# Opendigitalradio/ODR-DabMod

Hardware: AMD Instinct MI355X
Metric: Mode-I TX frames/sec (196608 IQ/frame) (higher is better)
Workload: dtype f32; 1 GPU; Mode I full chain from coded bits + GainControl(var) + FIRFilter(45 default taps), native 2.048 Msps (BASELINE config 3); mode=1, prewarm_steps=3, parallelism=1 independent streams

## Files before the change

odr-dabmod_amd/csrc/dabgpu_internal.h:

```cpp
#pragma once

#include <hip/hip_runtime.h>
#include <stddef.h>
#include <stdint.h>

namespace dabgpu {

constexpr int kMaxTaps = 128;
constexpr int kEqTaps = 160;
constexpr int kEqCentre = 56;
constexpr int kMaxTapsUnfused = 512;

struct Geometry {
    int mode;
    int nb_symbols;
    int K;
    int N;
    int logN;
    int null_size;
    int sym_size;
};

struct Tables {
    const float2 *twiddle;
    const uint16_t *src_carrier;
    const uint16_t *dst_pos;
    const uint8_t *phase_q;
    const float *mag;
    const float *taps;
    const float *window;
    const float2 *fir_h;
    const float *eq_g;
};

bool trace_on();
void trace_launch(const char *what);
#define DABGPU_LAUNCH(kernel, ...)                                      \
    do {                                                                \
        if (::dabgpu::trace_on()) ::dabgpu::trace_launch(#kernel);      \
        hipLaunchKernelGGL(kernel, __VA_ARGS__);                        \
    } while (0)

bool streams_overlap(hipStream_t a, hipStream_t b);
hipError_t create_stream_apart(const hipStream_t *others, int n, hipStream_t *out, bool *own);

struct GainParams {
    int mode;
    float constant;
    float var_variance;
    float var_c1;
    float var_c1_lo;
    float var_sq;
};

struct TfArgs {
    Geometry g;
    Tables t;
    GainParams gain;
    int ntaps;
    int n_frames;
    int chunks_per_frame;
    int syms_per_chunk;
    const uint8_t *bits;
    const float2 *carriers;
    float2 *out;
    size_t out_stride;
    float *gain1;
    const float2 *tii_seg;
    int tii_insert0;
    float cfr_clip, cfr_errclip;
    int cfr_mer_base;
    unsigned *cfr_counts;
    double *cfr_mer;
    double *cfr_papr;
    unsigned long long *clipped;
    int overlap;
    unsigned long long *phase_cycles;
};

enum TfFlags { TF_FROM_BITS = 1, TF_GAIN = 2, TF_GUARD = 4, TF_FIR = 8, TF_CFR = 16, TF_GVAR = 32 ,
               TF_OUT_S16 = 64, TF_WINDOW = 256, TF_EQ = 512, TF_OUT_U8 = 1024, TF_OUT_S8 = 2048 };
inline int tf_ofmt(unsigned flags) { return (flags & TF_OUT_S16) ? 1 : (flags & TF_OUT_U8) ? 2 : (flags & TF_OUT_S8) ? 3 : 0; }
inline unsigned tf_ofmt_flag(int fmt) { return fmt == 1 ? TF_OUT_S16 : fmt == 2 ? TF_OUT_U8 : fmt == 3 ? TF_OUT_S8 : 0u; }

hipError_t launch_tf(const TfArgs &a, unsigned flags, hipStream_t s);
size_t tf_lds_bytes(int logN, unsigned flags, int nt = 0, int overlap = 0, int ntaps = 0);
int tf_max_fused_taps();
bool tf_has_eq(const TfArgs &a, unsigned flags);
bool tf_small45(const TfArgs &a, unsigned flags);
bool tf_has_window(const TfArgs &a, unsigned flags);
bool tf_has_fmt(const TfArgs &a, unsigned flags);
bool tf_has_tii(const TfArgs &a, unsigned flags);

hipError_t launch_qpsk(const uint8_t *in, size_t nbytes, int K, float2 *out, hipStream_t s);
hipError_t launch_freq_interleave(const float2 *in, size_t nsamples, int K,
                                  const uint16_t *src_carrier, float2 *out, hipStream_t s);
hipError_t launch_phase_reference(const uint8_t *phase_q, int K, float2 *out, hipStream_t s);
hipError_t launch_diff_mod(const float2 *phase, const float2 *data, size_t nsym_data, int K,
                           float2 *out, hipStream_t s);
hipError_t launch_gain(const float2 *in, size_t nsym, int N, GainParams gp, float2 *out,
                       hipStream_t s);
hipError_t launch_gain_replay(float2 *x0, size_t n_frames, int nsym, int N, GainParams gp, float *gains, float *gain1,
                              bool apply, hipStream_t s);
hipError_t launch_guard_copy(const float2 *in, size_t n_frames, Geometry g, float2 *out,
                             hipStream_t s, const float *gains = nullptr);
hipError_t launch_guard_window(const float2 *in, size_t n_frames, Geometry g, int overlap,
                               const float *window, float2 *out, hipStream_t s, const float *gains = nullptr);
hipError_t launch_guard_fir(const float2 *in, size_t n_frames, Geometry g, int overlap, const float *window,
                            const float *taps, int ntaps, float2 *out, hipStream_t s, const float *gains = nullptr);
hipError_t launch_fir(const float2 *in, size_t frame_samples, size_t n_frames, const float *taps,
                      int ntaps, float2 *out, hipStream_t s);
hipError_t launch_poly(const float2 *in, size_t nsamples, const float *am, const float *pm,
                       float2 *out, hipStream_t s);
hipError_t launch_cic(const float2 *in, size_t nsamples, int K, const float *filter, float2 *out, hipStream_t s);
hipError_t launch_tii(const float2 *in, const uint8_t *acp, int K, int old_variant, int insert, float2 *out,
                      hipStream_t s);
hipError_t launch_tii_add(float2 *out, size_t stride, const float2 *seg, int seg_len, const float *gain1,
                          int insert0, size_t n_frames, hipStream_t s);
hipError_t launch_format(const float *in, size_t nfloats, int fmt, void *out, unsigned long long *clipped,
                         hipStream_t s);
hipError_t launch_lut(const float2 *in, size_t nsamples, float scale, const float *lut,
                      float2 *out, hipStream_t s);

constexpr int kFeCifBytes = 864 * 8;
constexpr int kFeHistory = 15;
struct FeUnit {
    uint32_t in_off, in_bytes;
    uint32_t out_bytes;
    uint32_t dst_off;
    int32_t owner;
    uint32_t nseg;
    uint32_t g0[6], base[6], pat[6];
};
struct FeArgs {
    const uint8_t *eti;
    const uint8_t *prbs;
    const FeUnit *units;
    const int16_t *owner;
    uint8_t *hist;
    uint8_t *fic;
    uint8_t *out;
    int n_eti, n_units, cifs, fic_out;
};
hipError_t launch_fe_encode(const FeArgs &a, hipStream_t s);
hipError_t launch_fe_assemble(const FeArgs &a, hipStream_t s);

struct ResamplerArgs {
    int nin, nout;
    float factor;
    const float *window;
    const float2 *tw_in;
    const float2 *tw_out;
    const float2 *in;
    const float2 *halo;
    float2 *halo_out;
    float2 *out;
    const float *poly;
    unsigned long long *clipped;
    size_t nhops;
    int L, M;
    const float2 *tw_s;
    const float2 *tw_l;
};
hipError_t launch_resampler(const ResamplerArgs &a, hipStream_t s);
bool resampler_has_s16(const ResamplerArgs &a);
// ... 4 lines not shown
```

odr-dabmod_amd/csrc/tf_kernel.h:

```cpp
#pragma once
#include <cstdio>
#include "device_common.h"
#include "tf_layout.h"

namespace dabgpu {
namespace {

constexpr unsigned kCX = 0x901Au;


template <int LOGN> struct ModeGeom;
template <> struct ModeGeom<11> { static constexpr int nb_symbols = 76, K = 1536, null_size = 2656, sym_size = 2552; };
template <> struct ModeGeom<9> { static constexpr int nb_symbols = 76, K = 384, null_size = 664, sym_size = 638; };
template <> struct ModeGeom<8> { static constexpr int nb_symbols = 153, K = 192, null_size = 345, sym_size = 319; };
template <> struct ModeGeom<10> { static constexpr int nb_symbols = 76, K = 768, null_size = 1328, sym_size = 1276; };

template <int LOGN, bool FROM_BITS, bool GAIN, bool GUARD, bool FIR, int NT, bool CFR = false, bool GVAR = false,
          bool ZONLY = false, int OFMT = 0, bool WIN = false, bool EQ = false>
__global__ __launch_bounds__((1 << LOGN) / 8 < 64 ? 64 : (1 << LOGN) / 8,
                             tf_variant(LOGN, FROM_BITS, GAIN, GUARD, FIR, NT, CFR, GVAR, OFMT, WIN, EQ).waves_per_simd)
void tf_kernel(const TfArgs a)
{
    static_assert(!GVAR || (GAIN && !FROM_BITS && !CFR), "GVAR is a specialisation of the carriers path with gain");
    static_assert(!CFR || GUARD == FIR || (FROM_BITS && GUARD),
                  "CFR variants: the full fused epilogue or none of it; the coded-bits chain also with the guard interval alone");
    static_assert(!ZONLY || (LOGN == 11 && GUARD && FIR && NT > 0 && !CFR),
                  "ZONLY: the dual transform of the Mode I chain with the fused FIR");
    static_assert(!ZONLY || FROM_BITS || GVAR || !GAIN, "ZONLY: no gain statistics over the time domain");
    static_assert(!WIN || (FROM_BITS && GUARD && (OFMT == 0 || EQ || (OFMT == 1 && !FIR && !CFR))),
                  "WIN: coded-bits chain with guard interval (integer store: every format with EQ, s16 without FIRFilter)");
    static_assert(!(WIN && FIR) || (!ZONLY && (NT == 0 || (NT == 45 && !CFR)) && !GVAR),
                  "WIN with FIR: the generic packed dual transform (all unfiltered samples at hand), run-time tap count -- or EQ");
    static_assert(!EQ || (FROM_BITS && GUARD && FIR && NT == 45 && !CFR && !GVAR && !ZONLY),
                  "EQ: the coded-bits chain with the 45-tap filter");
    static_assert(!EQ || LOGN == 11 || (LOGN == 10 && !WIN && OFMT == 0),
                  "EQ in transmission mode IV (round 6): complexf output, no windowing (Mode I: WIN with overlap <= kEqWinMax, every format)");
    typedef ModeGeom<LOGN> G;
    typedef Fft<LOGN> F;
    constexpr int N = F::N, T = F::T;
    constexpr TfVariant VAR = tf_variant(LOGN, FROM_BITS, GAIN, GUARD, FIR, NT, CFR, GVAR, OFMT, WIN, EQ);
    constexpr bool CFR_LEAN = VAR.cfr_lean, NOFIR_1BUF = VAR.nofir_1buf, DBUF = VAR.dbuf;
    (void)NOFIR_1BUF;
    constexpr bool HALVES = VAR.halves;
    constexpr int NH = HALVES ? 2 : 1;
    const int t_wg = threadIdx.x;
    const int half = HALVES ? (t_wg >> 5) : 0;
    const int t = HALVES ? (t_wg & 31) : t_wg;
    const bool lane_on = (HALVES || T >= 64) ? true : t < T;
    const unsigned long long on_mask = (HALVES || T >= 64) ? ~0ull : ((1ull << (T & 63)) - 1ull);
    const int tt = lane_on ? t : 0;
    auto hoff = [&](int n) __attribute__((always_inline)) -> int { return HALVES ? half * n : 0; };

    extern __shared__ __attribute__((aligned(16))) char smem[];
    cf *fbuf = reinterpret_cast<cf *>(smem);
    int fpar = 0;
    constexpr bool CFR_SEQ = VAR.cfr_seq;
    constexpr int kXElems = VAR.dual ? 2 * F::LDS_ELEMS : (DBUF ? 2 : 1) * F::LDS_ELEMS;
    double *red = reinterpret_cast<double *>(fbuf + NH * kXElems);
    fbuf += hoff(kXElems);
    uint32_t *phw = reinterpret_cast<uint32_t *>(red + NH * 16);
    red += hoff(16);
    cf *bnd = reinterpret_cast<cf *>(phw + NH * (GAIN ? (FROM_BITS ? T : 6 * T) : 0));
    phw += hoff(T);
    constexpr int KB = NT ? NT - 1 : kBnd;
    cf *wbuf = bnd;
    float *win_l = reinterpret_cast<float *>(wbuf + 6 * kWinMax);
    constexpr int kEqWm = (EQ && WIN) ? kEqWinMax : 0;
    constexpr int kEqQL = kEqTaps - 1 - kEqCentre + kEqWm, kEqQH = 43 + kEqCentre + kEqWm, kEqW = kEqWLen;
    static_assert(kEqQL + kEqQH + 1 + kEqWm <= kEqW && kEqTaps == 160, "EQ window (+ what the unused outputs of a narrower overlap read)");
    static_assert(kEqElems == 3 * kEqW + kEqDLen + (kEqTaps + 8) / 2 + 16 && 2 * kEqWinMax <= 32 && 2 * kEqWinMax + 44 <= 64,
                  "LDS share of the EQ variants (tf_lds_bytes)");
    cf *eq_zp = bnd, *eq_w = bnd + 2 * kEqW, *eq_d = eq_w + kEqW;
    float *g_l = reinterpret_cast<float *>(eq_d + kEqDLen);
    constexpr bool BWIN = VAR.bwin;
    constexpr int kBndElems = 4 * KB + (BWIN ? 4 : 0);
    uint32_t *bitbuf = reinterpret_cast<uint32_t *>(bnd + NH * (EQ ? kEqElems : (FIR && !WIN) ? kBndElems : ((WIN && !FIR) ? 7 * kWinMax : 0)));
    bnd += hoff(kBndElems);
    constexpr int kBitWords = (3 * N / 4) / 16;
    constexpr int kBitStride = kBitWords + 2;
    constexpr bool PAIR = VAR.pair;
    constexpr int kBitBlocks = PAIR ? 4 : 2;
    float *taps_l = reinterpret_cast<float *>(bitbuf + NH * (FROM_BITS ? kBitBlocks * kBitStride : 0));
    bitbuf += hoff(kBitBlocks * kBitStride);
    constexpr int kTapsL = VAR.bwin ? 0 : kMaxTaps, kMagL = 160;
    float *mag_l = taps_l + kTapsL;
    cf *unit8 = reinterpret_cast<cf *>(mag_l + kMagL);
    cf *tw8_l = unit8 + 64;
    F::fill_tw8(a.t.twiddle, tw8_l, t_wg);
    float *cfr_red = reinterpret_cast<float *>(tw8_l + 56);
    uint2 *bsh_l = reinterpret_cast<uint2 *>(cfr_red + 6 * ((T + 63) / 64));
    if (t_wg < 64) {
        const unsigned p = ((unsigned)t_wg + ((unsigned)t_wg >> 3)) & 7u;
        const float cx = (float)((int)((kCX >> (2u * p)) & 3u) - 1);
        const float cy = (float)((int)((kCX >> (2u * ((p + 6u) & 7u))) & 3u) - 1);
        unit8[t_wg] = mk(cx, cy);
    }
    for (int i = t_wg; i < kTapsL; i += blockDim.x) taps_l[i] = FIR ? a.t.taps[i] : 0.f;
    if (EQ)
        for (int i = t; i < kEqTaps + 8; i += blockDim.x) g_l[i] = i < kEqTaps ? a.t.eq_g[i] : 0.f;
    if (EQ) {
        for (int i = t; i < 3 * kEqW + kEqDLen; i += blockDim.x) eq_zp[i] = mk(0.f, 0.f);
    }
    const int W = WIN ? a.overlap : 0;
    constexpr bool kSkipTests = WIN && (FIR || OFMT != 0);
    constexpr int kWm = WIN ? (EQ ? kEqWinMax : (kWinMax < G::sym_size - N ? kWinMax : G::sym_size - N)) : 0;
    const int wfC = (WIN && FIR && !EQ) ? a.ntaps - 1 : 0, wfLP = wfC + 2 * W;
    cf *wfb = tw8_l + 56 + (CFR ? 3 * ((T + 63) / 64) : 0);
    cf *wf_cur = wfb + 2 * wfLP, *wf_U = wf_cur + (2 * W + wfC);
    if (WIN && FIR) win_l = EQ ? g_l + (kEqTaps + 8) : reinterpret_cast<float *>(wf_U + (2 * W + 2 * wfC));
    if (WIN)
        for (int i = t; i < 2 * W; i += blockDim.x) win_l[i] = a.t.window[i];
    if (FROM_BITS)
        for (int i = t_wg; i < G::nb_symbols; i += blockDim.x) mag_l[i] = a.t.mag[i];
    if (BWIN && t < 4) bnd[4 * KB + t] = mk(0.f, 0.f);
    lds_barrier();
    float4 tapa = make_float4(0.f, 0.f, 0.f, 0.f), tapb = tapa, tapc = tapa;
    if constexpr (BWIN) {
        const float4 *tp = reinterpret_cast<const float4 *>(a.t.taps + 12 * (t & 3));
        tapa = tp[0]; tapb = tp[1]; tapc = tp[2];
    }
    const float4 tapm = make_float4((t & 3) == 0 ? 1.f : 0.f, (t & 3) == 1 ? 1.f : 0.f, (t & 3) == 2 ? 1.f : 0.f, (t & 3) == 3 ? 1.f : 0.f);

    constexpr int K = G::K, nsym = G::nb_symbols + 1;
    const int frame0 = NH * (int)(blockIdx.x / a.chunks_per_frame);
    const int chunk = blockIdx.x - (frame0 / NH) * a.chunks_per_frame;
    const bool frame_ok = !HALVES || frame0 + half < a.n_frames;
    const int frame = HALVES ? min(frame0 + half, a.n_frames - 1) : frame0;
    const int s_begin = chunk * a.syms_per_chunk;
    const int s_end = chunk == a.chunks_per_frame - 1 ? nsym : min(nsym, s_begin + a.syms_per_chunk);
    constexpr bool TII_IN = FROM_BITS && GUARD && (EQ || !WIN) && !HALVES;
    const bool tii_on = TII_IN && a.tii_seg != nullptr && s_begin == 0 && (((frame & 1) == 0) == (a.tii_insert0 != 0));
    float g1s = 1.0f;
    if (frame0 >= a.n_frames || s_begin >= nsym) return;

    const int ntaps = NT ? NT : a.ntaps;
    const int C = FIR ? ntaps - 1 : 0;
    constexpr int cp0 = GUARD ? G::null_size - N : 0, cp = GUARD ? G::sym_size - N : 0;
    constexpr int len0 = N + cp0, len = N + cp;

    cf tw[F::NTW > 0 ? F::NTW : 1];
    F::template load_twiddles<true>(a.t.twiddle, tt, tw);

    const int r0 = (tt == 0) ? 3 : 0;
    int kpos[6];
    cf hk[6];
    cf hk8[CFR && FIR ? 8 : 1];
    {
        const int rr[6] = {r0, 1, 2, 5, 6, 7};
#pragma unroll
        for (int c = 0; c < 6; ++c) {
            const int bin = tt + T * rr[c];
            kpos[c] = (bin <= K / 2) ? bin - 1 : bin - N + K;
            if (FIR) hk[c] = a.t.fir_h[bin];
        }
    }
    if (CFR && FIR && !CFR_SEQ) {
#pragma unroll
        for (int m = 0; m < 8; ++m) hk8[m] = a.t.fir_h[tt + T * m];
    }
    int bitpos[6];
    unsigned bsh[6] = {0u, 0u, 0u, 0u, 0u, 0u};
    unsigned P = 0u;
    unsigned fpos[6] = {0u, 4u, 8u, tt == 0 ? 12u : 20u, tt == 0 ? 20u : 16u, tt == 0 ? 16u : 12u};
    const uint8_t *fbits = nullptr;
    if (FROM_BITS) {
        fbits = a.bits + (size_t)frame * (size_t)(G::nb_symbols - 1) * (size_t)(K / 4);
#pragma unroll
        for (int c = 0; c < 6; ++c) {
            bitpos[c] = a.t.src_carrier[kpos[c]];
            bsh[c] = (unsigned)bitpos[c] ^ 7u;
            P |= ((unsigned)a.t.phase_q[kpos[c]] & 3u) << fpos[c];
        }
        if constexpr (CFR_LEAN) {
#pragma unroll
            for (int j = 0; j < 3; ++j) bsh_l[j * T + t] = make_uint2(bsh[2 * j], bsh[2 * j + 1]);
        }
    }
    const cf *fcar = FROM_BITS ? nullptr
                               : a.carriers + (size_t)frame * (size_t)nsym * (size_t)K;
    constexpr int kOutBytes = OFMT == 0 ? 8 : (OFMT == 1 ? 4 : 2);
    const __amdgpu_buffer_rsrc_t orsrc = __builtin_amdgcn_make_buffer_rsrc(
        reinterpret_cast<char *>(a.out) + (size_t)frame0 * a.out_stride * kOutBytes, 0, (int)(NH * a.out_stride * kOutBytes), 0x00020000);
    const int hvoff = HALVES ? (frame_ok ? half * (int)a.out_stride : 0x07ffffff) : 0;
    unsigned nclip = 0;
    typedef unsigned v2u_ __attribute__((ext_vector_type(2)));
#ifdef DABGPU_STORE_AUX
    constexpr int kStoreAux = DABGPU_STORE_AUX;
#else
    constexpr int kStoreAux = (FROM_BITS && LOGN != 8) ? 2 : 0;
#endif
    auto put = [&](int soff, int voff, cf y) __attribute__((always_inline)) {
        if constexpr (OFMT == 1) {
            __builtin_amdgcn_raw_buffer_store_b32(s16_pack(y, nclip), orsrc, voff * 4, soff * 4, kStoreAux);
        } else if constexpr (OFMT == 2 || OFMT == 3) {
            __builtin_amdgcn_raw_buffer_store_b16(b8_pack<(OFMT == 3 ? 3 : 2)>(y, nclip), orsrc, voff * 2, soff * 2, kStoreAux);
        } else {
            const v2u_ d = {__builtin_bit_cast(unsigned, y.x), __builtin_bit_cast(unsigned, y.y)};
            __builtin_amdgcn_raw_buffer_store_b64(d, orsrc, (voff + hvoff) * 8, soff * 8, kStoreAux);
        }
    };

    auto advance = [&](const uint32_t *blk) __attribute__((always_inline)) {
        uint2 w[6];
        unsigned bs[6];
        if constexpr (CFR_LEAN) {
            int tl = t;
            asm volatile("" : "+v"(tl));
#pragma unroll
            for (int j = 0; j < 3; ++j) {
                const uint2 b2 = bsh_l[j * T + tl];
                bs[2 * j] = b2.x;
                bs[2 * j + 1] = b2.y;
            }
        } else {
#pragma unroll
            for (int c = 0; c < 6; ++c) bs[c] = bsh[c];
        }
#pragma unroll
        for (int c = 0; c < 6; ++c)
            w[c] = *reinterpret_cast<const uint2 *>(reinterpret_cast<const char *>(blk) + (__builtin_amdgcn_ubfe(bs[c], 5u, 6u) << 3));
        unsigned I = 0u, Q = 0u;
#pragma unroll
        for (int c = 0; c < 6; ++c) {
            I |= __builtin_amdgcn_ubfe(w[c].x, bs[c], 1u) << fpos[c];
            Q |= __builtin_amdgcn_ubfe(w[c].y, bs[c], 1u) << fpos[c];
        }
        P = (P + ((I ^ Q) | (Q << 1))) & 0x333333u;
    };
    auto fetch_block = [&](int d) __attribute__((always_inline)) -> uint32_t {
        const int dd = min(max(d, 0), G::nb_symbols - 2);
        int tf = t < kBitWords ? t : 0;
        if constexpr (CFR_LEAN) asm volatile("" : "+v"(tf));
        return reinterpret_cast<const uint32_t *>(fbits + (size_t)dd * (size_t)(K / 4))[tf];
    };
    const int bit_slot = t < kBitWords / 2 ? 2 * t : (t < kBitWords ? 2 * (t - kBitWords / 2) + 1 : kBitWords);

    static_assert(!PAIR || (T >= 2 * kBitWords && FROM_BITS), "PAIR: a lane per dword of two blocks");
    auto pair_lane = [&](int &b, int &j, int &slot) __attribute__((always_inline)) {
        int tl = t;
        asm volatile("" : "+v"(tl));
        b = (tl >= kBitWords && tl < 2 * kBitWords) ? 1 : 0;
        j = tl - b * kBitWords;
        slot = tl < 2 * kBitWords ? b * kBitStride + (j < kBitWords / 2 ? 2 * j : 2 * (j - kBitWords / 2) + 1) : kBitWords;
        if (tl >= 2 * kBitWords) j = 0;
    };
    auto fetch_pair = [&](int pr) __attribute__((always_inline)) -> uint32_t {
        int b, j, slot;
        pair_lane(b, j, slot);
        const int blk = min(max(2 * pr + b, 0), G::nb_symbols - 2);
        const uint32_t *src = reinterpret_cast<const uint32_t *>(fbits + (size_t)blk * (size_t)(K / 4)) + j;
        uint32_t w;
        asm volatile("global_load_dword %0, %1, off" : "=v"(w) : "v"(src));
        return w;
    };
    auto park_pair = [&](int pr, uint32_t w) __attribute__((always_inline)) {
        int b, j, slot;
        pair_lane(b, j, slot);
        asm volatile("s_waitcnt vmcnt(0)" : "+v"(w));
        bitbuf[2 * (pr & 1) * kBitStride + slot] = w;
    };

    constexpr bool MAG_IN_GAIN = EQ && GAIN;
    auto load_active = [&](int s, cf *val) __attribute__((always_inline)) {
        if (FROM_BITS) {
            const float mg = s >= 1 ? mag_l[s - 1] : 0.f;
#pragma unroll
            for (int c = 0; c < 6; ++c) {
                const unsigned rot64 = ((unsigned)(s - 1) & 7u) << 6;
                const cf u = *reinterpret_cast<const cf *>(reinterpret_cast<const char *>(unit8) +
                                                          ((__builtin_amdgcn_ubfe(P, fpos[c], 2u) << 4) | rot64));
                if (MAG_IN_GAIN) val[c] = u;
                else val[c] = s >= 1 ? mk(u.x * mg, u.y * mg) : mk(0.f, 0.f);
            }
        } else {
            const cf *sym = fcar + (size_t)min(s, nsym - 1) * (size_t)K + tt;
            val[0] = sym[(tt == 0 ? 3 * T : 0) - 1];
            val[1] = sym[T - 1];
            val[2] = sym[2 * T - 1];
            val[3] = sym[5 * T - N + K];
            val[4] = sym[6 * T - N + K];
            val[5] = sym[7 * T - N + K];
        }
    };
    const float m_r0 = r0 == 0 ? 1.0f : 0.0f, m_r3 = 1.0f - m_r0;
    auto place = [&](const cf *val, cf *v) __attribute__((always_inline)) {
        v[0] = cscale(val[0], m_r0);
        v[3] = cscale(val[0], m_r3);
        v[4] = mk(0.f, 0.f);
        v[1] = val[1]; v[2] = val[2]; v[5] = val[3]; v[6] = val[4]; v[7] = val[5];
    };

    if (FROM_BITS) {
        {
            const int nblk = s_begin - 2;
            constexpr int W = K / 32;
            constexpr int kThreadsTf = HALVES ? 32 : (T < 64 ? 64 : T);
            constexpr int NG = kThreadsTf / W;
            static_assert(K % 32 == 0 && NG >= 1 && (2 * NG + 2) * W * 4 <= kXElems * (int)sizeof(cf), "bit-sliced prefix");
            if (nblk > 0) {
                uint32_t *planes = reinterpret_cast<uint32_t *>(fbuf);
                const int j = t % W, g = t / W;
                uint32_t s0 = 0u, s1 = 0u;
                if (g < NG) {
                    const uint32_t *col = reinterpret_cast<const uint32_t *>(fbits) + j;
                    for (int b = g; b < nblk; b += NG) {
                        const uint32_t iw = col[(size_t)b * (K / 16)], qw = col[(size_t)b * (K / 16) + W];
                        const uint32_t l = iw ^ qw, c = s0 & l;
                        s0 ^= l;
                        s1 ^= qw ^ c;
                    }
                    planes[(2 * g) * W + j] = s0;
                    planes[(2 * g + 1) * W + j] = s1;
                }
                lds_barrier_vm();
                if (t < W) {
                    uint32_t a0 = planes[t], a1 = planes[W + t];
#pragma unroll
                    for (int gg = 1; gg < NG; ++gg) {
                        const uint32_t b0 = planes[(2 * gg) * W + t], b1 = planes[(2 * gg + 1) * W + t], c = a0 & b0;
                        a0 ^= b0;
                        a1 ^= b1 ^ c;
                    }
                    planes[2 * NG * W + t] = a0;
                    planes[(2 * NG + 1) * W + t] = a1;
                }
                lds_barrier();
                unsigned inc = 0u;
#pragma unroll
                for (int c = 0; c < 6; ++c) {
                    const unsigned n = (unsigned)bitpos[c], bit = 8u * ((n >> 3) & 3u) + 7u - (n & 7u);
                    const uint32_t lo = planes[2 * NG * W + (n >> 5)], hi = planes[(2 * NG + 1) * W + (n >> 5)];
                    inc |= (__builtin_amdgcn_ubfe(lo, bit, 1u) | (__builtin_amdgcn_ubfe(hi, bit, 1u) << 1)) << fpos[c];
                }
                P = (P + inc) & 0x333333u;
                lds_barrier();
            }
        }
        if constexpr (PAIR) {
            const int d_first = max(max(s_begin, 1) - 2, 0), p0 = d_first >> 1;
            park_pair(p0, fetch_pair(p0));
            if (d_first & 1) park_pair(p0 + 1, fetch_pair(p0 + 1));
        } else {
            bitbuf[bit_slot] = fetch_block(s_begin - 2);
        }
    }

    auto cfr_symbol = [&](cf *v, cf *zf, const cf *refv, int s, bool stats) __attribute__((always_inline)) {
        const float clip2 = a.cfr_clip * a.cfr_clip, eclip2 = a.cfr_errclip * a.cfr_errclip;
        const bool mer_sym = stats && s > 0 && s == (a.cfr_mer_base + frame) % nsym;
        constexpr int NW = (T + 63) / 64;
        constexpr bool KEEP_BEFORE = !CFR_LEAN;
        cf before[KEEP_BEFORE ? 8 : 1];
        float pk = 0.f, sm = 0.f;
        unsigned nclip = 0, neclip = 0;
#pragma unroll
        for (int m = 0; m < 8; ++m) {
            const float mag2 = v[m].x * v[m].x + v[m].y * v[m].y;
            pk = fmaxf(pk, mag2);
            sm += mag2;
            if (KEEP_BEFORE) before[m] = v[m];
            const bool over = mag2 > clip2;
            v[m] = cscale(v[m], over ? fabsf(a.cfr_clip) * fast_rsq(mag2) : 1.0f);
            nclip += over ? 1u : 0u;
        }
        if (stats) {
            pk = lane_on ? pk : 0.f; sm = lane_on ? sm : 0.f;
            wave_max_sum_dpp(pk, sm);
            if ((t & 63) == 0) { cfr_red[2 * (t >> 6)] = pk; cfr_red[2 * (t >> 6) + 1] = sm; }
        }
        F::template run<-1, DBUF, cf, true>(v, fbuf, fpar, tw, tt, tw8_l);
        if (stats && t == 0) {
            float p = 0.f;
            double q = 0.;
#pragma unroll
            for (int w = 0; w < NW; ++w) { p = fmaxf(p, cfr_red[2 * w]); q += (double)cfr_red[2 * w + 1]; }
            double *pp = a.cfr_papr + ((size_t)frame * nsym + s) * 4;
            pp[0] = (double)p;
            pp[1] = q / (double)N;
        }
        cf rv[CFR_LEAN ? 8 : 1];
        if constexpr (CFR_LEAN) {
            cf val2[6];
            load_active(s, val2);
            place(val2, rv);
            refv = rv;
        }
#pragma unroll
        for (int m = 0; m < 8; ++m) {
            const cf c = cscale(v[m], 1.0f / (float)N);
            cf e = csub(refv[m], c);
            const float mag2 = e.x * e.x + e.y * e.y;
            const bool over = mag2 > eclip2;
            const float f = over ? fabsf(a.cfr_errclip) * fast_rsq(mag2) : 1.0f;
            neclip += over ? 1u : 0u;
            v[m] = mk(fmaf(e.x, f, c.x), fmaf(e.y, f, c.y));
        }
        if constexpr (CFR_SEQ) {
            cf hh[8];
            int tl = tt;
            asm volatile("" : "+v"(tl));
#pragma unroll
            for (int m = 0; m < 8; ++m) hh[m] = a.t.fir_h[tl + T * m];
#pragma unroll
            for (int m = 0; m < 8; ++m) zf[m] = cmul(v[m], hh[m]);
            F::template run<+1, DBUF, cf, true>(zf, fbuf, fpar, tw, tt, tw8_l);
            F::template run<+1, DBUF, cf, true>(v, fbuf, fpar, tw, tt, tw8_l);
        } else if (FIR) {
            c2 v2[8];
#pragma unroll
            for (int m = 0; m < 8; ++m) {
                const cf f = cmul(v[m], hk8[CFR && FIR ? m : 0]);
                v2[m] = c2{make_float2(v[m].x, f.x), make_float2(v[m].y, f.y)};
            }
            F::template run<+1, DBUF, c2, true>(v2, reinterpret_cast<c2 *>(fbuf), fpar, tw, tt, tw8_l);
#pragma unroll
            for (int m = 0; m < 8; ++m) {
                v[m] = mk(v2[m].re.x, v2[m].im.x);
                zf[m] = mk(v2[m].re.y, v2[m].im.y);
            }
        } else {
            F::template run<+1, DBUF, cf, true>(v, fbuf, fpar, tw, tt, tw8_l);
        }
        if (stats) {
            float c1 = lane_on ? (float)nclip : 0.f, c2_ = lane_on ? (float)neclip : 0.f;
// ... 339 lines not shown
            for (int u = 0; u < 10; ++u)
#pragma unroll
                for (int r = 0; r < kEqR; ++r) acc[r] = axpy(acc[r], gg[u], wv[r + 9 - u]);
        }
#define DABGPU_DPP6(CTRL)                                                                       \
        "v_add_f32_dpp %0, %0, %0 " CTRL " row_mask:0xf bank_mask:0xf\n\t"                      \
        "v_add_f32_dpp %1, %1, %1 " CTRL " row_mask:0xf bank_mask:0xf\n\t"                      \
        "v_add_f32_dpp %2, %2, %2 " CTRL " row_mask:0xf bank_mask:0xf\n\t"                      \
        "v_add_f32_dpp %3, %3, %3 " CTRL " row_mask:0xf bank_mask:0xf\n\t"                      \
        "v_add_f32_dpp %4, %4, %4 " CTRL " row_mask:0xf bank_mask:0xf\n\t"                      \
        "v_add_f32_dpp %5, %5, %5 " CTRL " row_mask:0xf bank_mask:0xf\n\t"
#define DABGPU_DPP2(CTRL)                                                                       \
        "v_add_f32_dpp %6, %6, %6 " CTRL " row_mask:0xf bank_mask:0xf\n\t"                      \
        "v_add_f32_dpp %7, %7, %7 " CTRL " row_mask:0xf bank_mask:0xf\n\t"
        asm volatile("s_nop 1\n\t"
                     DABGPU_DPP6("quad_perm:[1,0,3,2]") DABGPU_DPP2("quad_perm:[1,0,3,2]")
                     DABGPU_DPP6("quad_perm:[2,3,0,1]") DABGPU_DPP2("quad_perm:[2,3,0,1]")
                     DABGPU_DPP6("row_ror:4") DABGPU_DPP2("row_ror:4") DABGPU_DPP6("row_ror:8") DABGPU_DPP2("row_ror:8")
                     : "+v"(acc[0].x), "+v"(acc[0].y), "+v"(acc[1].x), "+v"(acc[1].y), "+v"(acc[2].x), "+v"(acc[2].y),
                       "+v"(acc[3].x), "+v"(acc[3].y));
#undef DABGPU_DPP6
#undef DABGPU_DPP2
        if (t < kEqLanes && (t & 15) == 0) {
#pragma unroll
            for (int r = 0; r < kEqR; ++r) eq_d[44 * cur + kEqR * (t >> 4) + r] = acc[r];
        }
        if (t >= kEqLanes && t < kEqLanes + 44) eq_d[88 + 44 * cur + (t - kEqLanes)] = zp[kEqQL - C + (t - kEqLanes)];
        if (pb_pos >= 0 && t < kEqLanes) eq_store_pending(ypend);
        pb_pos = prev_pos + prev_seg - C;
    };
    auto eq_boundary_flush = [&]() __attribute__((always_inline)) {
        if (pb_pos < 0) return;
        lds_barrier();
        eq_store_pending(eq_step2_pending(cur ^ 1));
        pb_pos = -1;
    };

    auto eq_boundary_small = [&](const cf *zp) __attribute__((always_inline)) {
        constexpr int kEqR = 4, kEqLanes = 16 * ((44 + kEqR - 1) / kEqR);
        constexpr int kEqThreads = T < 64 ? 64 : T;
#pragma unroll
        for (int eq_base = 0; eq_base < kEqLanes; eq_base += kEqThreads) {
            const int tj = eq_base + t;
            cf acc[4] = {mk(0.f, 0.f), mk(0.f, 0.f), mk(0.f, 0.f), mk(0.f, 0.f)};
            if (tj < kEqLanes) {
                const int m0 = kEqR * (tj >> 4), j0 = 10 * (tj & 15);
                const cf *wp = eq_w + (m0 + (kEqTaps - 1 - 9) - j0);
                const float2 *g2 = reinterpret_cast<const float2 *>(g_l + j0);
                cf wv[kEqR + 9];
                float gg[10];
#pragma unroll
                for (int i = 0; i < kEqR + 9; ++i) wv[i] = wp[i];
#pragma unroll
                for (int u = 0; u < 5; ++u) { const float2 g = g2[u]; gg[2 * u] = g.x; gg[2 * u + 1] = g.y; }
#pragma unroll
                for (int u = 0; u < 10; ++u)
#pragma unroll
                    for (int r = 0; r < kEqR; ++r) acc[r] = axpy(acc[r], gg[u], wv[r + 9 - u]);
            }
#pragma unroll
            for (int r = 0; r < kEqR; ++r) row16_sum2_dpp(acc[r].x, acc[r].y);
            if (tj < kEqLanes && (tj & 15) == 0) {
#pragma unroll
                for (int r = 0; r < kEqR; ++r) eq_d[kEqR * (tj >> 4) + r] = acc[r];
            }
        }
        lds_barrier();
#pragma unroll
        for (int eq_base = 0; eq_base < 4 * 44; eq_base += kEqThreads) {
            const int tj = eq_base + t;
            const int i = min(tj >> 2, C - 1), q = tj & 3;
            const float *tq = taps_l + (C - i) + q;
            const cf *dq = eq_d + q;
            cf y = mk(0.f, 0.f);
#pragma unroll
            for (int k = 0; k < 11; ++k) y = axpy(y, tq[4 * k], dq[4 * k]);
            quad_sum2_dpp(y.x, y.y);
            y = cadd(y, zp[kEqQL - C + i]);
            if (tj < 4 * C && q == 0) put(prev_pos + prev_seg - C, tj >> 2, y);
        }
    };

    int bb = 0;
    cf nval[6];
    if (!FROM_BITS) load_active(s_begin, nval);

    int s_loop = s_begin;
    if (FROM_BITS && s_begin == 0) {
        const int nz = len0 - C - W;
        if (!tii_on)
            for (int i0 = 0; i0 < nz; i0 += kThreads)
                if (i0 + t < nz) put(i0, t, mk(0.f, 0.f));
        if (EQ) {
            for (int i = t; i < kEqW; i += (int)blockDim.x) eq_zp[cur * kEqW + i] = mk(0.f, 0.f);
        } else if (FIR && !WIN) {
            for (int i = t; i < KB; i += (HALVES ? 32 : (int)blockDim.x)) bnd[cur * 2 * KB + i] = mk(0.f, 0.f);
        }
        if (FIR) {
            have_prev = true;
            prev_pos = 0;
            prev_seg = len0;
        }
        if (WIN && FIR && !EQ) {
            for (int i = t; i < wfLP; i += (int)blockDim.x) wfb[cur * wfLP + i] = mk(0.f, 0.f);
        } else if (WIN && !FIR) {
            for (int i = t; i < 2 * W; i += (int)blockDim.x) wbuf[cur * 2 * kWinMax + i] = mk(0.f, 0.f);
            have_prev = true;
        }
        s_loop = 1;
    }

    PhaseTimer pt;
    unsigned pt_iterations = 0;
    pt.begin();
    for (int s = s_loop; s < s_stop; ++s) {
        if (FROM_BITS) __builtin_assume(s >= 1);
        pt.stamp(PH_LOOP);
        ++pt_iterations;
        const bool lookahead = s >= s_end;
        cf val[6], v[8];
        uint32_t pf = 0u;
        if (FROM_BITS) {
            lds_barrier();
            if constexpr (PAIR) {
                if (s >= 2) advance(bitbuf + ((s - 2) & 3) * kBitStride);
                if ((s & 1) == 0) pf = fetch_pair(s >> 1);
            } else {
                if (s >= 2) advance(bitbuf + bb * kBitStride);
                pf = fetch_block(s - 1);
            }
            load_active(s, val);
            if (GAIN && !CFR && a.gain.mode == 2) {
                phw[tt] = P >> 12;
                lds_barrier();
                const unsigned o = phw[(T - tt) & (T - 1)];
                const unsigned sums = P + o + (((unsigned)(s - 1) & 3u) * 0x111u);
                int cnt = 0, cnt_hi = 0;
#pragma unroll
                for (int j = 0; j < 3; ++j) {
                    const unsigned f = sums & (3u << (4 * j));
                    const unsigned long long b0 = __builtin_amdgcn_uicmp(f, 0u, 32), b2 = __builtin_amdgcn_uicmp(f, 2u << (4 * j), 32);
                    if constexpr (HALVES) {
                        cnt += __builtin_popcount((unsigned)b0) - __builtin_popcount((unsigned)b2);
                        cnt_hi += __builtin_popcount((unsigned)(b0 >> 32)) - __builtin_popcount((unsigned)(b2 >> 32));
                    } else {
                        cnt += __builtin_popcountll(b0 & on_mask);
                        cnt -= __builtin_popcountll(b2 & on_mask);
                    }
                }
                const float part = (float)((HALVES && half) ? cnt_hi : cnt);
                float *redf = reinterpret_cast<float *>(red + 8 * (s & 1));
                if ((t & 63) == 0) redf[WIN ? __builtin_amdgcn_readfirstlane(t >> 6) : t >> 6] = part;
            }
        } else {
#pragma unroll
            for (int c = 0; c < 6; ++c) val[c] = nval[c];
            if (s + 1 < s_stop) load_active(s + 1, nval);
            if (GAIN && !CFR && (GVAR || a.gain.mode == 2) && s > 0)
                spectral_partial(val, reinterpret_cast<float *>(red + 8 * (s & 1)));
        }
        constexpr bool DUAL = FIR && !EQ;
        cf z[8];
        cf uedge = mk(0.f, 0.f);
        if (DUAL && CFR) {
            place(val, v);
            F::template run<+1, DBUF, cf, true>(v, fbuf, fpar, tw, tt, tw8_l);
            if constexpr (CFR_SEQ) {
                cfr_symbol(v, z, nullptr, s, !lookahead);
            } else {
                cf refv[8];
                place(val, refv);
                cfr_symbol(v, z, refv, s, !lookahead);
            }
        } else if (DUAL) {
            cf valf[6];
#pragma unroll
            for (int c = 0; c < 6; ++c) valf[c] = cmul(val[c], hk[c]);
            place(val, v);
            place(valf, z);
            c2 v2[8];
#pragma unroll
            for (int r = 0; r < 8; ++r) v2[r] = c2{make_float2(v[r].x, z[r].x), make_float2(v[r].y, z[r].y)};
            if constexpr (ZONLY) {
                F::template run_dual_zonly<+1>(v2, reinterpret_cast<c2 *>(fbuf), tw, tt, tw8_l, z, uedge);
            } else {
                F::template run<+1, DBUF, c2, true>(v2, reinterpret_cast<c2 *>(fbuf), fpar, tw, tt, tw8_l);
#pragma unroll
                for (int m = 0; m < 8; ++m) {
                    v[m] = mk(v2[m].re.x, v2[m].im.x);
                    z[m] = mk(v2[m].re.y, v2[m].im.y);
                }
            }
        } else {
            if (EQ) {
#pragma unroll
                for (int c = 0; c < 6; ++c) val[c] = cmul(val[c], hk[c]);
            }
            place(val, v);
            pt.stamp(PH_INPUT);
            F::template run<+1, DBUF, cf, true>(v, fbuf, fpar, tw, tt, tw8_l, &pt);
            if constexpr (CFR_LEAN) {
                cfr_symbol(v, z, nullptr, s, !lookahead);
            } else if (CFR) {
                cf refv[8];
                place(val, refv);
                cfr_symbol(v, z, refv, s, !lookahead);
            }
        }

        if (FROM_BITS) {
            if constexpr (PAIR) {
                if ((s & 1) == 0) park_pair(s >> 1, pf);
            } else {
                bitbuf[(bb ^ 1) * kBitStride + bit_slot] = pf;
            }
        }

        float g = 1.0f;
        if (GAIN) {
            bool g_final = false;
            if (FROM_BITS && !CFR && a.gain.mode == 2) {
                const float *redf = reinterpret_cast<const float *>(red + 8 * (s & 1));
                float S = 0.f;
#pragma unroll
                for (int w = 0; w < (T + 63) / 64; ++w) S += redf[w];
                const float mg = mag_l[s - 1];
                const float par1 = (float)(1u + ((unsigned)(s - 1) & 1u));
                const float m2 = mg * mg * par1;
                const float A = (float)(K / 2) + fabsf(S);
                const float u = MAG_IN_GAIN ? par1 * A : A;
                float r = fast_rsq(u);
                r = fmaf(0.5f * r, fmaf(-u * r, r, 1.0f), r);
                const float dlt = MAG_IN_GAIN ? 0.f
                                  : (par1 == 1.0f ? 1.0f - mg : fmaf(-mg, 2.4203e-8f, fmaf(-mg, 1.41421354f, 1.0f)));
                const bool blank = m2 * fmaxf((float)(K / 2) + S, 0.f) * a.gain.var_sq < 1.0f;
                const float lo = (MAG_IN_GAIN && WIN) ? a.gain.var_c1_lo : fmaf(a.gain.var_c1, dlt, a.gain.var_c1_lo);
                g = blank ? a.gain.constant * (MAG_IN_GAIN ? mg : 1.0f) : fmaf(a.gain.var_c1, r, lo * r);
                g_final = true;
            } else if (!FROM_BITS && !CFR && (GVAR || a.gain.mode == 2) && s > 0) {
                g = spectral_gain(reinterpret_cast<const float *>(red + 8 * (s & 1)));
            } else if (GVAR) {
                g = g_null;
            } else if (ZONLY || EQ) {
                g = 512.0f;
            } else {
                g = (s == 0) ? g_null : symbol_gain_fused<T>(v, a.gain, red + 8 * (s & 1), tt, lane_on);
            }
            if (!g_final) g = g * a.gain.constant;
            if (FROM_BITS && a.gain1 != nullptr && s == 1 && t == 0) a.gain1[frame] = g;
            if (TII_IN && s == 1) g1s = __builtin_bit_cast(float, __builtin_amdgcn_readfirstlane(__builtin_bit_cast(int, g)));
            if (MAG_IN_GAIN && !g_final) g *= mag_l[s - 1];
        }

        constexpr bool PRESCALED = (DUAL || WIN || EQ) && GAIN;
        if (((WIN && !FIR) || EQ) && GAIN) {
#pragma unroll
            for (int m = 0; m < 8; ++m) v[m] = cscale(v[m], g);
        } else if (PRESCALED && ZONLY) {
            uedge = cscale(uedge, g);
#pragma unroll
            for (int m = 0; m < 8; ++m) z[m] = cscale(z[m], g);
        } else if (PRESCALED) {
#pragma unroll
            for (int m = 0; m < 8; ++m) {
                const float2 re = make_float2(v[m].x, z[m].x) * g, im = make_float2(v[m].y, z[m].y) * g;
                v[m] = mk(re.x, im.x);
                z[m] = mk(re.y, im.y);
            }
        }
        auto scaled = [&](cf x) __attribute__((always_inline)) -> cf {
            return (PRESCALED || !GAIN) ? x : cscale(x, g);
        };

        const int cpl = (!FROM_BITS && s == 0) ? cp0 : cp;
        const int seg = N + cpl;
        const int pos = GUARD ? (s == 0 ? 0 : len0 + (s - 1) * len) : s * N;
        if constexpr (EQ) {
            cf *zp_prev = eq_zp + cur * kEqW, *zp_new = eq_zp + (cur ^ 1) * kEqW;
            [[maybe_unused]] constexpr int n0 = (N - cp) - kEqQL;
            if constexpr (LOGN == 11) {
                static_assert(LOGN != 11 || (n0 >= 5 * T && n0 + kEqQL + kEqQH < 7 * T && kEqQL < T && kEqQH < T), "EQ windows: slots 5, 6, 7, 0");
                if (t >= n0 - 5 * T) { const int iw = t - (n0 - 5 * T); eq_w[iw] = csub(v[5], zp_prev[iw]); }
                if (t <= n0 + kEqQL + kEqQH - 6 * T) { const int iw = t + (6 * T - n0); eq_w[iw] = csub(v[6], zp_prev[iw]); }
                if (t >= T - kEqQL) zp_new[t - (T - kEqQL)] = v[7];
                if (t <= kEqQH) zp_new[kEqQL + t] = v[0];
            } else if (lane_on) {
                static_assert(kEqQL + kEqQH + 1 <= N && kEqQH < N - kEqQL, "EQ windows: one period holds them");
#pragma unroll
                for (int m = 0; m < 8; ++m) {
                    const int n = t + T * m;
                    int q = n - (N - cp);
                    if (q > kEqQH) q -= N;
                    if (q < -kEqQL) q += N;
                    if (q >= -kEqQL && q <= kEqQH) eq_w[q + kEqQL] = csub(v[m], zp_prev[q + kEqQL]);
                    if (m * T <= kEqQH && n <= kEqQH) zp_new[kEqQL + n] = v[m];
// ... 362 lines not shown
```

odr-dabmod_amd/csrc/tf_launch.hip:

```cpp
#include "tf_layout.h"

#include <algorithm>

namespace dabgpu {

hipError_t launch_tf_8_0(const TfArgs &a, unsigned flags, hipStream_t s);
hipError_t launch_tf_9_0(const TfArgs &a, unsigned flags, hipStream_t s);
hipError_t launch_tf_10_0(const TfArgs &a, unsigned flags, hipStream_t s);
hipError_t launch_tf_11_0(const TfArgs &a, unsigned flags, hipStream_t s);
hipError_t launch_tf_11_45(const TfArgs &a, unsigned flags, hipStream_t s);
hipError_t launch_tf_8_45(const TfArgs &a, unsigned flags, hipStream_t s);
hipError_t launch_tf_9_45(const TfArgs &a, unsigned flags, hipStream_t s);
hipError_t launch_tf_10_45(const TfArgs &a, unsigned flags, hipStream_t s);

size_t tf_lds_bytes(int logN, unsigned flags, int nt, int overlap, int ntaps)
{
    const size_t N = (size_t)1 << logN;
    const bool eq = flags & TF_EQ;

    const TfVariant v = tf_variant(logN, flags & TF_FROM_BITS, flags & TF_GAIN, flags & TF_GUARD, flags & TF_FIR, nt, flags & TF_CFR,
                                   flags & TF_GVAR, tf_ofmt(flags), flags & TF_WINDOW, eq);
    const bool cfr_lean = v.cfr_lean, dbuf = v.dbuf, dual = v.dual;
    const size_t nh = v.halves ? 2 : 1;
    size_t b = dual ? (N + N / 8) * 2 * sizeof(float2) : (dbuf ? 2 : 1) * (N + N / 8) * sizeof(float2);
    b += 16 * sizeof(double);
    if (flags & TF_GAIN) b += ((flags & TF_FROM_BITS) ? 1 : 6) * (N / 8) * sizeof(uint32_t);
    const bool wf = (flags & TF_WINDOW) && (flags & TF_FIR) && !eq;
    if (eq) b += kEqElems * sizeof(float2);
    else if ((flags & TF_FIR) && !wf) b += (4 * (nt ? nt - 1 : kBnd) + (v.bwin ? 4 : 0)) * sizeof(float2);
    if (flags & TF_FROM_BITS) b += (v.pair ? 4 : 2) * ((3 * N / 4) / 16 + 2) * sizeof(uint32_t);
    b *= nh;
    b += ((v.bwin ? 0 : kMaxTaps) + 160) * sizeof(float) + 64 * sizeof(float2);
    b += 56 * sizeof(float2);
    if (flags & TF_CFR) b += 6 * ((N / 8 + 63) / 64) * sizeof(float);
    if (cfr_lean) b += 3 * (N / 8) * 2 * sizeof(uint32_t);
    if (wf) {
        const size_t C = (size_t)std::max(ntaps - 1, 0), W = (size_t)std::max(overlap, 0);
        b += (2 * (C + 2 * W) + (2 * W + C) + (2 * W + 2 * C)) * sizeof(float2) + 2 * W * sizeof(float) + 16;
    } else if ((flags & TF_WINDOW) && !eq) {
        b += 7 * kWinMax * sizeof(float2);
    }
    return b;
}

bool tf_has_window(const TfArgs &a, unsigned flags)
{
    const unsigned want = TF_FROM_BITS | TF_GUARD;
    if ((flags & want) != want || a.overlap < 1 || a.overlap > kWinMax) return false;
    if (flags & TF_FIR)
        return a.ntaps >= 1 && a.ntaps <= kBnd && a.ntaps <= kMaxTaps &&
               a.overlap + a.ntaps - 1 <= a.g.sym_size - a.g.N;
    return a.overlap <= a.g.sym_size - a.g.N;
}

int tf_max_fused_taps() { return kBnd < kMaxTaps ? kBnd : kMaxTaps; }

bool tf_small45(const TfArgs &a, unsigned flags)
{
    const unsigned want = TF_FROM_BITS | TF_GUARD | TF_FIR;
    if (a.g.logN == 8 && (flags & TF_GAIN) && a.gain.mode == 1) return false;
    return a.g.logN >= 8 && a.g.logN <= 10 && a.ntaps == 45 && (flags & ~(unsigned)(TF_GAIN | TF_EQ)) == want;
}

bool tf_has_eq(const TfArgs &a, unsigned flags)
{
    const unsigned want = TF_FROM_BITS | TF_GUARD | TF_FIR;
    if ((flags & TF_WINDOW) && (a.overlap < 1 || a.overlap > kEqWinMax)) return false;
    if (a.g.logN != 11 && ((flags & TF_WINDOW) || tf_ofmt(flags))) return false;
    return a.t.eq_g != nullptr && a.g.logN >= 10 && a.g.logN <= 11 && a.ntaps == 45 && (flags & want) == want && !(flags & TF_CFR) &&
           (!(flags & TF_GAIN) || a.gain.mode != 1);
}

bool tf_has_tii(const TfArgs &a, unsigned flags)
{
    const unsigned want = TF_FROM_BITS | TF_GUARD;
    if ((flags & want) != want || a.syms_per_chunk < 2) return false;
    if (flags & TF_WINDOW) return (flags & TF_EQ) && tf_has_eq(a, flags);
    return (flags & TF_EQ) ? tf_has_eq(a, flags) : true;
}

bool tf_has_fmt(const TfArgs &a, unsigned flags)
{
    const int of = tf_ofmt(flags);
    if (!of || a.g.logN != 11 || (flags & (TF_FROM_BITS | TF_GUARD)) != (TF_FROM_BITS | TF_GUARD)) return false;
    if (flags & TF_WINDOW) {
        if (flags & TF_CFR) return false;
        return (flags & TF_FIR) ? ((flags & TF_EQ) && tf_has_eq(a, flags)) : of == 1;
    }
    if (flags & TF_CFR) return of == 1;
    if (!(flags & TF_FIR)) return true;
    if (of == 1) return true;
    return (flags & TF_EQ) && a.ntaps == 45 && (!(flags & TF_GAIN) || a.gain.mode != 1);
}

hipError_t launch_tf(const TfArgs &a, unsigned flags, hipStream_t s)
{
    if (flags & TF_FIR) {
        const int C = a.ntaps - 1;
        if (a.ntaps < 1 || a.ntaps > kMaxTaps || a.ntaps > kBnd || C > a.g.sym_size - a.g.N)
            return hipErrorInvalidValue;
    }
    switch (a.g.logN) {
        case 8: return tf_small45(a, flags) ? launch_tf_8_45(a, flags, s) : launch_tf_8_0(a, flags, s);
        case 9: return tf_small45(a, flags) ? launch_tf_9_45(a, flags, s) : launch_tf_9_0(a, flags, s);
        case 10: return tf_small45(a, flags) ? launch_tf_10_45(a, flags, s) : launch_tf_10_0(a, flags, s);
        case 11:
            return ((flags & TF_FIR) && a.ntaps == 45 && !((flags & TF_CFR) && (flags & TF_WINDOW))) ? launch_tf_11_45(a, flags, s)
                                                       : launch_tf_11_0(a, flags, s);
    }
    return hipErrorInvalidValue;
}

}
```

odr-dabmod_amd/csrc/tf_layout.h:

```cpp
#pragma once
#include "dabgpu_internal.h"

namespace dabgpu {
constexpr int kEqWinMax = 10;
constexpr int kEqWLen = 240, kEqDLen = 176;
constexpr int kEqElems = 3 * kEqWLen + kEqDLen + (kEqTaps + 8) / 2 + 16;
constexpr int kWinMax = 128;
constexpr int kBnd = 128;

struct TfVariant {
    bool cfr_lean;
    bool cfr_seq;
    bool nofir_1buf;
    bool dbuf;
    bool dual;
    bool halves;
    bool bwin;
    bool pair;
    int waves_per_simd;
};
constexpr TfVariant tf_variant(int logn, bool from_bits, bool gain, bool guard, bool fir, int nt, bool cfr, bool gvar,
                               int ofmt, bool win, bool eq)
{
    TfVariant v{};
    v.cfr_lean = cfr && logn == 11 && from_bits && guard && !win && (!fir || nt == 45);
    v.cfr_seq = v.cfr_lean && fir;
    v.nofir_1buf = logn == 11 && from_bits && guard && !fir && !cfr && (!win || ofmt != 0);
    v.dbuf = !fir && !v.cfr_lean && !v.nofir_1buf;
    v.dual = fir && !eq && !v.cfr_seq;
    v.bwin = logn != 11 && fir && nt == 45 && !cfr && !win && !eq;
    v.halves = logn == 8 && from_bits && guard && fir && nt == 45 && !cfr && !gvar && ofmt == 0 && !win && !eq;
    v.pair = eq && logn == 11;
    v.waves_per_simd = eq ? (logn == 11 ? 4 : 3)
                       : cfr ? (v.cfr_lean ? 4 : ((from_bits && guard && !(win && fir)) ? 3 : 2))
                       : !fir ? (v.nofir_1buf ? ((win || (ofmt == 3 && !gain)) ? 4 : 5) : 2)
                       : (gvar ? 3 : ((gain && !from_bits) ? 2 : 3));
    return v;
}
}
```

Before: 2.788 million frames/s.

## Prefetch coded bits in groups of symbols straight into an LDS ring

In the EQ/pair Mode I transform path, the bit fetch now loads a group of 14 symbols at a time directly into an LDS ring using global_load_lds_dword. Before, it loaded one pair per two symbols into registers and then stored them to LDS after a wait. This cuts the per-symbol vmcnt waits and the register round trip, and spreads the fetch across four waves. The cost is a larger LDS ring, which static_asserts keep within four workgroups per CU. The inline asm juggling M0 is fragile.

```diff
diff --git a/odr-dabmod_amd/csrc/dabgpu_internal.h b/odr-dabmod_amd/csrc/dabgpu_internal.h
--- a/odr-dabmod_amd/csrc/dabgpu_internal.h
+++ b/odr-dabmod_amd/csrc/dabgpu_internal.h
@@ -80,7 +80,7 @@
 
 enum TfFlags { TF_FROM_BITS = 1, TF_GAIN = 2, TF_GUARD = 4, TF_FIR = 8, TF_CFR = 16, TF_GVAR = 32 ,
                TF_OUT_S16 = 64, TF_WINDOW = 256, TF_EQ = 512, TF_OUT_U8 = 1024, TF_OUT_S8 = 2048 };
-inline int tf_ofmt(unsigned flags) { return (flags & TF_OUT_S16) ? 1 : (flags & TF_OUT_U8) ? 2 : (flags & TF_OUT_S8) ? 3 : 0; }
+constexpr int tf_ofmt(unsigned flags) { return (flags & TF_OUT_S16) ? 1 : (flags & TF_OUT_U8) ? 2 : (flags & TF_OUT_S8) ? 3 : 0; }
 inline unsigned tf_ofmt_flag(int fmt) { return fmt == 1 ? TF_OUT_S16 : fmt == 2 ? TF_OUT_U8 : fmt == 3 ? TF_OUT_S8 : 0u; }
 
 hipError_t launch_tf(const TfArgs &a, unsigned flags, hipStream_t s);
diff --git a/odr-dabmod_amd/csrc/tf_kernel.h b/odr-dabmod_amd/csrc/tf_kernel.h
--- a/odr-dabmod_amd/csrc/tf_kernel.h
+++ b/odr-dabmod_amd/csrc/tf_kernel.h
@@ -79,9 +79,10 @@
     constexpr int kBitWords = (3 * N / 4) / 16;
     constexpr int kBitStride = kBitWords + 2;
     constexpr bool PAIR = VAR.pair;
-    constexpr int kBitBlocks = PAIR ? 4 : 2;
-    float *taps_l = reinterpret_cast<float *>(bitbuf + NH * (FROM_BITS ? kBitBlocks * kBitStride : 0));
-    bitbuf += hoff(kBitBlocks * kBitStride);
+    constexpr int GRP = VAR.group, kRing = PAIR ? GRP + 2 : 0;
+    constexpr int kBitElems = PAIR ? kRing * kBitWords : 2 * kBitStride;
+    float *taps_l = reinterpret_cast<float *>(bitbuf + NH * (FROM_BITS ? kBitElems : 0));
+    bitbuf += hoff(kBitElems);
     constexpr int kTapsL = VAR.bwin ? 0 : kMaxTaps, kMagL = 160;
     float *mag_l = taps_l + kTapsL;
     cf *unit8 = reinterpret_cast<cf *>(mag_l + kMagL);
@@ -235,30 +236,30 @@
     };
     const int bit_slot = t < kBitWords / 2 ? 2 * t : (t < kBitWords ? 2 * (t - kBitWords / 2) + 1 : kBitWords);
 
-    static_assert(!PAIR || (T >= 2 * kBitWords && FROM_BITS), "PAIR: a lane per dword of two blocks");
-    auto pair_lane = [&](int &b, int &j, int &slot) __attribute__((always_inline)) {
+    static_assert(!PAIR || (T == 256 && kBitWords == 96 && FROM_BITS && GRP % 2 == 0 && (kRing & (kRing - 1)) == 0),
+                  "PAIR: three 64-lane pieces per pair of blocks, four waves, a power-of-two ring");
+    auto fetch_pairs = [&](int p0, int np) __attribute__((always_inline)) {
+        const int wv = __builtin_amdgcn_readfirstlane(t >> 6);
         int tl = t;
         asm volatile("" : "+v"(tl));
-        b = (tl >= kBitWords && tl < 2 * kBitWords) ? 1 : 0;
-        j = tl - b * kBitWords;
-        slot = tl < 2 * kBitWords ? b * kBitStride + (j < kBitWords / 2 ? 2 * j : 2 * (j - kBitWords / 2) + 1) : kBitWords;
-        if (tl >= 2 * kBitWords) j = 0;
-    };
-    auto fetch_pair = [&](int pr) __attribute__((always_inline)) -> uint32_t {
-        int b, j, slot;
-        pair_lane(b, j, slot);
-        const int blk = min(max(2 * pr + b, 0), G::nb_symbols - 2);
-        const uint32_t *src = reinterpret_cast<const uint32_t *>(fbits + (size_t)blk * (size_t)(K / 4)) + j;
-        uint32_t w;
-        asm volatile("global_load_dword %0, %1, off" : "=v"(w) : "v"(src));
-        return w;
-    };
-    auto park_pair = [&](int pr, uint32_t w) __attribute__((always_inline)) {
-        int b, j, slot;
-        pair_lane(b, j, slot);
-        asm volatile("s_waitcnt vmcnt(0)" : "+v"(w));
-        bitbuf[2 * (pr & 1) * kBitStride + slot] = w;
-    };
+        tl &= 63;
+        const unsigned ring = (unsigned)(uintptr_t)(__attribute__((address_space(3))) uint32_t *)bitbuf;
+#pragma unroll 1
+        for (int k = wv; k < 3 * np; k += 4) {
+            const int i = k / 3, c = k - 3 * i;
+            const int q = 64 * c + tl;
+            const int b = q >= kBitWords ? 1 : 0, r = q - b * kBitWords;
+            const int blk = min(max(2 * (p0 + i) + b, 0), G::nb_symbols - 2);
+            const uint32_t *src = reinterpret_cast<const uint32_t *>(fbits + (size_t)blk * (size_t)(K / 4)) +
+                                  ((r & 1) * (kBitWords / 2) + (r >> 1));
+            const unsigned dst = __builtin_amdgcn_readfirstlane(
+                ring + (unsigned)((((p0 + i) & (kRing / 2 - 1)) * 2 * kBitWords + 64 * c) * 4));
+            unsigned keep;
+            asm volatile("s_mov_b32 %0, m0\n\ts_mov_b32 m0, %2\n\ts_nop 0\n\tglobal_load_lds_dword %1, off\n\ts_mov_b32 m0, %0"
+                         : "=&s"(keep) : "v"(src), "s"(dst) : "memory");
+        }
+    };
+    auto wait_pairs = [&]() __attribute__((always_inline)) { asm volatile("s_waitcnt vmcnt(0)" ::: "memory"); };
 
     constexpr bool MAG_IN_GAIN = EQ && GAIN;
     auto load_active = [&](int s, cf *val) __attribute__((always_inline)) {
@@ -337,9 +338,14 @@
             }
         }
         if constexpr (PAIR) {
-            const int d_first = max(max(s_begin, 1) - 2, 0), p0 = d_first >> 1;
-            park_pair(p0, fetch_pair(p0));
-            if (d_first & 1) park_pair(p0 + 1, fetch_pair(p0 + 1));
+            const int s_first = max(s_begin, 1), d_first = max(s_first - 2, 0), g0 = d_first / GRP;
+            if ((g0 + 1) * GRP < s_first) {
+                fetch_pairs((g0 + 1) * (GRP / 2) - 1, 1);
+                fetch_pairs((g0 + 1) * (GRP / 2), GRP / 2);
+            } else {
+                fetch_pairs(g0 * (GRP / 2), GRP / 2);
+            }
+            wait_pairs();
         } else {
             bitbuf[bit_slot] = fetch_block(s_begin - 2);
         }
@@ -845,6 +851,7 @@
     };
 
     int bb = 0;
+    [[maybe_unused]] int s_fetch = 0;
     cf nval[6];
     if (!FROM_BITS) load_active(s_begin, nval);
 
@@ -873,6 +880,7 @@
         s_loop = 1;
     }
 
+    if constexpr (PAIR) s_fetch = (s_loop + GRP - 1) / GRP * GRP;
     PhaseTimer pt;
     unsigned pt_iterations = 0;
     pt.begin();
@@ -882,12 +890,17 @@
         ++pt_iterations;
         const bool lookahead = s >= s_end;
         cf val[6], v[8];
-        uint32_t pf = 0u;
+        [[maybe_unused]] uint32_t pf = 0u;
+        [[maybe_unused]] bool fetched = false;
         if (FROM_BITS) {
             lds_barrier();
             if constexpr (PAIR) {
-                if (s >= 2) advance(bitbuf + ((s - 2) & 3) * kBitStride);
-                if ((s & 1) == 0) pf = fetch_pair(s >> 1);
+                if (s >= 2) advance(bitbuf + ((s - 2) & (kRing - 1)) * kBitWords);
+                fetched = s == s_fetch;
+                if (fetched) {
+                    fetch_pairs(s >> 1, GRP / 2);
+                    s_fetch += GRP;
+                }
             } else {
                 if (s >= 2) advance(bitbuf + bb * kBitStride);
                 pf = fetch_block(s - 1);
@@ -973,7 +986,7 @@
 
         if (FROM_BITS) {
             if constexpr (PAIR) {
-                if ((s & 1) == 0) park_pair(s >> 1, pf);
+                if (fetched) wait_pairs();
             } else {
                 bitbuf[(bb ^ 1) * kBitStride + bit_slot] = pf;
             }
diff --git a/odr-dabmod_amd/csrc/tf_launch.hip b/odr-dabmod_amd/csrc/tf_launch.hip
--- a/odr-dabmod_amd/csrc/tf_launch.hip
+++ b/odr-dabmod_amd/csrc/tf_launch.hip
@@ -13,7 +13,8 @@
 hipError_t launch_tf_9_45(const TfArgs &a, unsigned flags, hipStream_t s);
 hipError_t launch_tf_10_45(const TfArgs &a, unsigned flags, hipStream_t s);
 
-size_t tf_lds_bytes(int logN, unsigned flags, int nt, int overlap, int ntaps)
+namespace {
+constexpr size_t lds_bytes(int logN, unsigned flags, int nt, int overlap, int ntaps)
 {
     const size_t N = (size_t)1 << logN;
     const bool eq = flags & TF_EQ;
@@ -28,7 +29,7 @@
     const bool wf = (flags & TF_WINDOW) && (flags & TF_FIR) && !eq;
     if (eq) b += kEqElems * sizeof(float2);
     else if ((flags & TF_FIR) && !wf) b += (4 * (nt ? nt - 1 : kBnd) + (v.bwin ? 4 : 0)) * sizeof(float2);
-    if (flags & TF_FROM_BITS) b += (v.pair ? 4 : 2) * ((3 * N / 4) / 16 + 2) * sizeof(uint32_t);
+    if (flags & TF_FROM_BITS) b += (v.pair ? (v.group + 2) * ((3 * N / 4) / 16) : 2 * ((3 * N / 4) / 16 + 2)) * sizeof(uint32_t);
     b *= nh;
     b += ((v.bwin ? 0 : kMaxTaps) + 160) * sizeof(float) + 64 * sizeof(float2);
     b += 56 * sizeof(float2);
@@ -42,6 +43,18 @@
     }
     return b;
 }
+
+constexpr unsigned kPairFlags = TF_FROM_BITS | TF_GUARD | TF_FIR | TF_EQ;
+constexpr size_t kLdsPerCu = 160 * 1024;
+static_assert(tf_variant(11, true, true, true, true, 45, false, false, 0, false, true).pair &&
+              tf_variant(11, true, true, true, true, 45, false, false, 0, false, true).group == kTfGroup, "the variants meant below");
+static_assert(lds_bytes(11, kPairFlags | TF_GAIN, 45, 0, 45) <= kLdsPerCu / 4 && lds_bytes(11, kPairFlags, 45, 0, 45) <= kLdsPerCu / 4 &&
+              lds_bytes(11, kPairFlags | TF_GAIN | TF_WINDOW, 45, kEqWinMax, 45) <= kLdsPerCu / 4 &&
+              lds_bytes(11, kPairFlags | TF_GAIN | TF_OUT_S16, 45, 0, 45) <= kLdsPerCu / 4,
+              "group prefetch: the ring must leave four workgroups' LDS on a CU");
+}
+
+size_t tf_lds_bytes(int logN, unsigned flags, int nt, int overlap, int ntaps) { return lds_bytes(logN, flags, nt, overlap, ntaps); }
 
 bool tf_has_window(const TfArgs &a, unsigned flags)
 {
diff --git a/odr-dabmod_amd/csrc/tf_layout.h b/odr-dabmod_amd/csrc/tf_layout.h
--- a/odr-dabmod_amd/csrc/tf_layout.h
+++ b/odr-dabmod_amd/csrc/tf_layout.h
@@ -17,8 +17,14 @@
     bool halves;
     bool bwin;
     bool pair;
+    int group;
     int waves_per_simd;
 };
+#ifndef DABGPU_TF_GROUP
+#define DABGPU_TF_GROUP 14
+#endif
+constexpr int kTfGroup = DABGPU_TF_GROUP;
+static_assert(kTfGroup >= 2 && kTfGroup % 2 == 0 && ((kTfGroup + 2) & (kTfGroup + 1)) == 0, "group + 2: a power of two");
 constexpr TfVariant tf_variant(int logn, bool from_bits, bool gain, bool guard, bool fir, int nt, bool cfr, bool gvar,
                                int ofmt, bool win, bool eq)
 {
@@ -31,6 +37,7 @@
     v.bwin = logn != 11 && fir && nt == 45 && !cfr && !win && !eq;
     v.halves = logn == 8 && from_bits && guard && fir && nt == 45 && !cfr && !gvar && ofmt == 0 && !win && !eq;
     v.pair = eq && logn == 11;
+    v.group = v.pair ? kTfGroup : 0;
     v.waves_per_simd = eq ? (logn == 11 ? 4 : 3)
                        : cfr ? (v.cfr_lean ? 4 : ((from_bits && guard && !(win && fir)) ? 3 : 2))
                        : !fir ? (v.nofir_1buf ? ((win || (ofmt == 3 && !gain)) ? 4 : 5) : 2)
```

Result: no change. 2.790 million frames/s (median of 2 runs) (+0.1%).
